# BartvLaatum/GreenLight-Gym2

Measured on AMD Instinct MI355X. Metric: TomatoEnv env-steps/sec, higher is better.
Workload: dtype f32

## Files before the change

greenlight-gym2_amd/csrc/glgym.hip:

```cpp
#include <hip/hip_runtime.h>

#include <cmath>
#include <cstdio>
#include <cstdlib>
#include <cstring>
#include <new>
#include <string>
#include <type_traits>
#include <vector>

#include "glgym.h"
#include "gl_model.hpp"
#include "gl_model_quad.hpp"
#include "gl_reward.hpp"
#include "gl_step_select.hpp"
#include "glgym_bdf.h"
#include "glgym_rng.h"
#include "glgym_plan.h"

using namespace glm;

namespace {

thread_local std::string g_err;

#define HIPCHK(expr)                                                                                   \
    do {                                                                                               \
        hipError_t e_ = (expr);                                                                        \
        if (e_ != hipSuccess) {                                                                        \
            g_err = std::string(#expr) + ": " + hipGetErrorString(e_);                                 \
            return GLGYM_EHIP;                                                                         \
        }                                                                                              \
    } while (0)

constexpr int WAVE = 64;

#include "gl_default_const.inc"
static_assert(sizeof(ModelConst<float>) == sizeof(kDefaultConstF32_image), "regenerate gl_default_const.inc");
static_assert(sizeof(ModelConst<double>) == sizeof(kDefaultConstF64_image), "regenerate gl_default_const.inc");
template <class T> struct DefaultConst;
template <> struct DefaultConst<float> {
    static constexpr ModelConst<float> value = __builtin_bit_cast(ModelConst<float>, kDefaultConstF32_bits);
};
template <> struct DefaultConst<double> {
    static constexpr ModelConst<double> value = __builtin_bit_cast(ModelConst<double>, kDefaultConstF64_bits);
};
__constant__ const ModelConst<float> g_default_f32 = __builtin_bit_cast(ModelConst<float>, kDefaultConstF32_bits);
__constant__ const ModelConst<double> g_default_f64 = __builtin_bit_cast(ModelConst<double>, kDefaultConstF64_bits);
template <class T> __device__ __forceinline__ const ModelConst<T>& device_default();
template <> __device__ __forceinline__ const ModelConst<float>& device_default<float>() { return g_default_f32; }
template <> __device__ __forceinline__ const ModelConst<double>& device_default<double>() { return g_default_f64; }

template <class T> struct RewardConst : RewardConstBase<T> {};

template <class T> struct StepArgsT {
    int B, ld;
    T* x; T* u;
    const float* action; const T* control;
    const T* weather; int weather_rows;
    const int* w_off; int* timestep;
    const T* crop_p;
    int N;
    T* reward; T* info; unsigned char* done; float* metrics; int* step_flags;
    T dt; int n_sub;
    T gasR, tCanMin;
    int nd;
    float du, u_min[NU], u_max[NU];
    int verify;
    int pipe;
    int window;
};

template <class T> __device__ __forceinline__ T wave_sum(T v)
{
#pragma unroll
    for (int o = 32; o > 0; o >>= 1) v += __shfl_xor(v, o, WAVE);
    return v;
}

constexpr int OBS_NCORE = 23;
__device__ __forceinline__ float obs_core_feature(int j, float prim, float aux, float sday, int ts, double doy_inc, double hod_inc)
{
#pragma clang fp contract(off)
    const float kPpm = (float)(8.3144598 / (101325.0 * 44.01e-3));
    const int k = ts > 0 ? ts - 1 : 0;
    const float sat = 610.78f * __builtin_amdgcn_exp2f(1.44269504f * 17.2694f * aux * __builtin_amdgcn_rcpf(aux + 238.3f));
    const float rh = fminf(fmaxf(100.0f * prim * __builtin_amdgcn_rcpf(sat), 0.0f), 100.0f);
    const float ppm = kPpm * (aux + 273.15f) * prim;
    const int c = j - 18;
    const double rev = (c <= 2) ? __builtin_fma((double)ts, doy_inc, (double)sday) * (1.0 / 365.0)
                                : (double)ts * hod_inc * (1.0 / 24.0);
    const float fr = (float)(rev - floor(rev));
    const float clk = (c == 1 || c == 3) ? __builtin_amdgcn_sinf(fr) : __builtin_amdgcn_cosf(fr);
    float v = prim;
    v = (j == 0 || j == 16) ? ppm : v;
    v = (j == 2 || j == 15) ? rh : v;
    v = (j == 18) ? (float)k : v;
    v = (j > 18) ? clk : v;
    return v;
}
__device__ __forceinline__ constexpr int obs_core_module(int j) { return j < 4 ? 0 : j < 7 ? 1 : j < 13 ? 2 : j < 18 ? 3 : 4; }
__device__ __forceinline__ constexpr int obs_core_col(int j) { return j < 4 ? j : j < 7 ? j - 4 : j < 13 ? j - 7 : j < 18 ? j - 13 : j - 18; }

__device__ __forceinline__ void philox4x32_10(unsigned c0, unsigned c1, unsigned c2, unsigned c3, unsigned k0,
                                              unsigned k1, unsigned* out)
{
#pragma unroll
    for (int r = 0; r < 10; ++r) {
        const unsigned long long p0 = 0xD2511F53ull * c0, p1 = 0xCD9E8D57ull * c2;
        const unsigned n0 = (unsigned)(p1 >> 32) ^ c1 ^ k0, n1 = (unsigned)p1;
        const unsigned n2 = (unsigned)(p0 >> 32) ^ c3 ^ k1, n3 = (unsigned)p0;
        c0 = n0; c1 = n1; c2 = n2; c3 = n3;
        k0 += 0x9E3779B9u; k1 += 0xBB67AE85u;
    }
    out[0] = c0; out[1] = c1; out[2] = c2; out[3] = c3;
}

template <class T>
__device__ __forceinline__ void reset_env(int b, int ld, T* x, T* u, int* timestep, const T* weather, int weather_rows, int* w_off,
                                          const int* start_rows, const float* start_days, int n_starts, float* start_day, int* episode,
                                          unsigned long long seed, int nd)
{
#pragma clang fp contract(off)
    if (start_rows && n_starts > 0) {
        const int ep = episode ? episode[b] : 0;
        unsigned rnd[4];
        philox4x32_10((unsigned)b, (unsigned)ep, 0x5eedu, 0u, (unsigned)seed, (unsigned)(seed >> 32), rnd);
        const int j = (int)(rnd[0] % (unsigned)n_starts);
        w_off[b] = start_rows[j];
        if (start_day && start_days) start_day[b] = start_days[j];
        if (episode) episode[b] = ep + 1;
    }
    int r = w_off[b];
    r = r < 0 ? 0 : (r >= weather_rows ? weather_rows - 1 : r);
    const double co2Out = (double)weather[(size_t)r * nd + 3], tSoOut = (double)weather[(size_t)r * nd + 6];
    const double tAir = 16.5;
    double xi[NX];
    xi[0] = xi[1] = co2Out;
    for (int i = 2; i <= 10; ++i) xi[i] = tAir;
    xi[4] = tAir + 4;
    xi[11] = 0.25 * (3.0 * tAir + tSoOut);
    xi[12] = 0.25 * __builtin_fma(2.0, tSoOut, 2.0 * tAir);
    xi[13] = 0.25 * __builtin_fma(3.0, tSoOut, tAir);
    xi[14] = tSoOut;
    xi[15] = xi[16] = 90.0 / 100.0 * (610.78 * exp(17.2694 * tAir / (tAir + 238.3)));
    xi[17] = xi[18] = xi[19] = xi[20] = tAir;
    xi[21] = xi[4];
    xi[22] = 0.0; xi[23] = 9.5283e4; xi[24] = 2.5107e5; xi[25] = 5.5338e4; xi[26] = 3.0978e3; xi[27] = 0.0;
    for (int i = 0; i < NX; ++i) x[(size_t)i * ld + b] = T(xi[i]);
    for (int j = 0; j < NU; ++j) u[(size_t)j * ld + b] = T(0);
    timestep[b] = 0;
}

#ifndef GL_OBS_ROWS
#define GL_OBS_ROWS 16
#endif
constexpr int OBS_ROWS = GL_OBS_ROWS, OBS_MAX_NP = 128;
struct StepObsArgs {
    float* obs; const float* start_day;
    double doy_inc, hod_inc;
    int Np, dim, moff[6];
};
constexpr int STEP_OBS_MAX_DIM_OCC2 = WAVE * ((2 * NX + GL_N_SLOW) | 1) / OBS_ROWS, STEP_OBS_MAX_DIM_OCC1 = 512;
struct StepNoObs {};
struct StepObsResetArgs : StepObsArgs {
    float* term_obs;
    int* w_off_rw; float* start_day_rw; int* episode;
    const int* start_rows; const float* start_days; int n_starts;
    unsigned long long seed;
};
constexpr int GL_SCH_OBS = 8;
constexpr int GL_SCH_RESET = 16;
template <int EPI> struct StepObsSel { using type = StepNoObs; };
template <> struct StepObsSel<GL_SCH_OBS> { using type = StepObsArgs; };
template <> struct StepObsSel<GL_SCH_OBS | GL_SCH_RESET> { using type = StepObsResetArgs; };

#ifndef GL_STEP_WAVES_PER_SIMD
#define GL_STEP_WAVES_PER_SIMD 1
#endif
#ifndef GL_RK4_WIN_F32
#define GL_RK4_WIN_F32 4
#endif
#ifndef GL_RK4_WIN_F64
#define GL_RK4_WIN_F64 4
#endif
template <class T> struct RK4_WINDOW { static constexpr int value = sizeof(T) == 4 ? GL_RK4_WIN_F32 : GL_RK4_WIN_F64; };
constexpr int gl_order(int sch) { return sch == 0 ? 4 : sch == 1 ? 2 : sch == 2 ? 3 : 5; }
template <class T, int SCH> struct SchemeWin { static constexpr int value = SCH == 0 ? RK4_WINDOW<T>::value : SCH == 1 ? 4 : SCH == 2 ? 3 : 2; };

template <class T, bool PER_ENV_CROP, bool DEFAULT_P, bool PIPE = false, int SCHX = 0, int OCC = GL_STEP_WAVES_PER_SIMD>
__global__ __launch_bounds__(WAVE, OCC) void step_kernel(StepArgsT<T> a, ModelConst<T> m_arg, RewardConst<T> rw,
                                                         typename StepObsSel<(SCHX & (GL_SCH_OBS | GL_SCH_RESET))>::type o)
{
    constexpr bool OBS = (SCHX & GL_SCH_OBS) != 0, RST = (SCHX & GL_SCH_RESET) != 0;
    constexpr int SCH = SCHX & (GL_SCH_OBS - 1);
    static_assert(!OBS || (sizeof(T) == 4 && !PIPE), "observation epilogue: fp32, default ODE");
    static_assert(!RST || (OBS && !PER_ENV_CROP), "auto-reset epilogue: behind the observation epilogue, shared crop parameters");
    const ModelConst<T>& m = DEFAULT_P ? device_default<T>() : m_arg;
    constexpr bool WBUF = OCC == 2;
    constexpr int WSTRIDE = (2 * NX + GL_N_SLOW) | 1;
    alignas(16) __shared__ float sh_w[WBUF ? WAVE * WSTRIDE : WAVE * NU];
    float* sh_act = sh_w;
    const int lane = threadIdx.x;
    const int b0 = blockIdx.x * WAVE;
    const int b = b0 + lane;
    const bool live = b < a.B;
    const int bb = live ? b : a.B - 1;

    T u[NU];
    if (a.action) {
        const int n_tile = min(WAVE, a.B - b0) * NU;
        for (int i = lane; i < n_tile; i += WAVE) sh_act[i] = a.action[(size_t)b0 * NU + i];
        __syncthreads();
        const int l = live ? lane : (a.B - 1 - b0);
#pragma unroll
        for (int j = 0; j < NU; ++j) {
            const float inc = sh_act[l * NU + j] * a.du;
            const T v = a.u[(size_t)j * a.ld + bb] + T(inc);
            u[j] = Math<T>::min(Math<T>::max(v, T(a.u_min[j])), T(a.u_max[j]));
        }
    } else {
#pragma unroll
        for (int j = 0; j < NU; ++j) u[j] = a.control[(size_t)j * a.ld + bb];
    }

    T x0[NX];
#pragma unroll
    for (int i = 0; i < NX; ++i) x0[i] = a.x[(size_t)i * a.ld + bb];
    const int ts = a.timestep[bb];
    int row = a.w_off[bb] + ts;
    row = row < 0 ? 0 : (row >= a.weather_rows ? a.weather_rows - 1 : row);
    T d[7];
#pragma unroll
    for (int j = 0; j < 7; ++j) d[j] = a.weather[(size_t)row * a.nd + j];

    CropConst<T> crLocal;
    if (PER_ENV_CROP) {
        T pc[NCROP];
#pragma unroll
        for (int i = 0; i < NCROP; ++i) pc[i] = a.crop_p[(size_t)i * a.ld + bb];
        make_crop_const<T, T>(pc, a.gasR, a.tCanMin, crLocal);
    }
    const CropConst<T>& cr = PER_ENV_CROP ? crLocal : m.crop;
    StepCoef<T> s_reg;
    precompute(u, d, m, cr, s_reg);
    if (PIPE) {
        const T tPipe = a.weather[(size_t)row * a.nd + 10], swOff = a.weather[(size_t)row * a.nd + 12];
        s_reg.pipeTrack = ((tPipe < T(1)) || (swOff > T(0))) ? T(0) : T(1);
        s_reg.tPipeSet = tPipe;
    }
    const StepCoef<T>& s = s_reg;
    if (live) {
#pragma unroll
        for (int j = 0; j < NU; ++j) a.u[(size_t)j * a.ld + b] = u[j];
    }
    T del_reg[WBUF ? 1 : NX];
    T* wb = reinterpret_cast<T*>(sh_w) + (size_t)lane * WSTRIDE;
    T* del = WBUF ? wb + NX + GL_N_SLOW : del_reg;
    if (WBUF) {
        __syncthreads();
#pragma unroll
        for (int i = 0; i < NX; ++i) wb[i] = x0[i];
        wb[5] = x0[3] - x0[5]; wb[7] = x0[2] - x0[7]; wb[20] = x0[2] - x0[20]; wb[6] = x0[5] - x0[6];
    }
    bool bad;
    int extra_steps, first_flags = 0;
    const int retries = rk4_delta_guarded<T, PIPE, gl_order(SCH), SchemeWin<T, SCH>::value, WBUF>(x0, s, m, cr, a.dt, a.n_sub, del, &bad, &extra_steps, a.verify != 0, &first_flags, a.window, wb);
    const T uBoil = a.u[(size_t)0 * a.ld + bb], uCo2 = a.u[(size_t)1 * a.ld + bb], uLamp = a.u[(size_t)4 * a.ld + bb];
    if (WBUF) {
#pragma unroll
        for (int i = 0; i < NX; ++i) x0[i] = a.x[(size_t)i * a.ld + bb];
    }

    T x1[NX];
#pragma unroll
    for (int i = 0; i < NX; ++i) x1[i] = bad ? x0[i] : x0[i] + del[i];
    {
        const double per_step = (double)a.dt / 86400.0;
        double t_start = (double)x0[NX - 1] - (double)ts * per_step;
        if (fabs(t_start) < 5e-4) t_start = 0.0;
        if (!bad) x1[NX - 1] = T(t_start + ((double)ts + 1.0) * per_step);
    }

    const T co2ppm = rw.kPpm * (x1[2] + T(273.15)) * x1[0];
    const T rh = Math<T>::min(Math<T>::max(T(100) * x1[15] / sat_vp_exact(x1[2]), T(0)), T(100));
    const T o3[3] = {co2ppm, x1[2], rh};
    T viol[3], pen = T(0);
#pragma unroll
    for (int i = 0; i < 3; ++i) {
        viol[i] = Math<T>::max(rw.lo[i] - o3[i], T(0)) + Math<T>::max(o3[i] - rw.hi[i], T(0));
        pen += viol[i] * rw.invMaxViol[i];
    }
    const T heat = uBoil * rw.heatK, elec = uLamp * rw.elecK, co2c = uCo2 * rw.co2K;
    const T varc = heat + co2c + elec;
    const T gains = (bad ? T(0) : del[25]) * rw.gainK;
    const T profit = gains - varc;
    const T reward = (profit - rw.minProfit) * rw.invRange - pen;
    const bool term = bad || (ts >= a.N);

    if (live) {
#pragma unroll
        for (int i = 0; i < NX; ++i) a.x[(size_t)i * a.ld + b] = x1[i];
        a.timestep[b] = ts + 1;
        a.reward[b] = reward;
        a.done[b] = term ? 1 : 0;
        if (a.step_flags) a.step_flags[b] = first_flags | (retries << 8) | (bad ? GLGYM_SF_FAILED : 0) | (min(extra_steps, 32767) << 16);
        if (a.info) {
            const T inf[GLGYM_NINFO] = {profit, gains, varc, rw.fixedCosts, co2c, heat, elec, viol[1], viol[0], viol[2], T(0)};
#pragma unroll
            for (int i = 0; i < GLGYM_NINFO; ++i) a.info[(size_t)i * a.ld + b] = inf[i];
        }
    }
    if (a.metrics) {
        const float w = live ? 1.f : 0.f;
        float mv[GLGYM_NMETRIC] = {w * (float)reward, w * (float)profit, (live && term) ? 1.f : 0.f,
                                   (live && bad) ? 1.f : 0.f, w * (float)viol[0], w * (float)viol[1],
                                   w * (float)viol[2], w, w * (float)retries, w * (float)extra_steps,
                                   (live && (first_flags & SC_FLAG_ERR)) ? 1.f : 0.f, (live && (first_flags & SC_FLAG_BRANCH)) ? 1.f : 0.f,
                                   (live && (first_flags & (SC_FLAG_CAP | SC_FLAG_NONFINITE))) ? 1.f : 0.f,
                                   (live && (first_flags & 16)) ? 1.f : 0.f};
        float* mrep = a.metrics + (size_t)(blockIdx.x % GLGYM_METRIC_REPLICAS) * GLGYM_METRIC_STRIDE;
#pragma unroll
        for (int i = 0; i < GLGYM_NMETRIC; ++i) {
            const float sum = wave_sum(mv[i]);
            if (lane == 0) atomicAdd(mrep + i, sum);
        }
    }
    if constexpr (OBS) {
        typedef float v4f __attribute__((ext_vector_type(4)));
        float* span;
        if constexpr (WBUF) {
            span = sh_w;
        } else {
            __shared__ float4 sh_obs4[OBS_ROWS * STEP_OBS_MAX_DIM_OCC1 / 4];
            span = reinterpret_cast<float*>(sh_obs4);
        }
        const int dim = o.dim;
        const int ts1 = ts + 1;
        const int base = a.w_off[bb] + (ts1 > 0 ? ts1 - 1 : 0);
        const int basec = base >= a.weather_rows ? a.weather_rows - 1 : (base < 0 ? 0 : base);
        const T* wrow = a.weather + (size_t)basec * a.nd;
        float wv[5];
#pragma unroll
        for (int j = 0; j < 5; ++j) wv[j] = wrow[j];
        const float sday = o.start_day[bb];
        const float uo[NU] = {uBoil, uCo2, a.u[(size_t)2 * a.ld + bb], a.u[(size_t)3 * a.ld + bb], uLamp, a.u[(size_t)5 * a.ld + bb]};
        float f[OBS_NCORE];
#pragma unroll
        for (int j = 0; j < OBS_NCORE; ++j) {
            const int xi = j == 0 ? 0 : j == 1 ? 2 : j == 2 ? 15 : j == 3 ? 9 : j == 4 ? 21 : j == 5 ? 25 : 26;
            const float prim = j < 7 ? x1[xi] : (j < 13 ? uo[(j >= 7 && j < 13) ? j - 7 : 0] : wv[j < 18 ? j - 13 : 0]);
            const float aux = j < 13 ? x1[2] : wv[1];
            f[j] = obs_core_feature(j, prim, aux, sday, ts1, o.doy_inc, o.hod_inc);
        }
        const int n_live = min(WAVE, a.B - b0);
        const int nf = o.moff[5] >= 0 ? 5 * o.Np : 0;
        __syncthreads();
        for (int s0 = 0; s0 < n_live; s0 += OBS_ROWS) {
            const int nrows = min(OBS_ROWS, n_live - s0);
            const int r_me = lane - s0;
            if (r_me >= 0 && r_me < nrows) {
#pragma unroll
                for (int j = 0; j < OBS_NCORE; ++j) {
                    const int mo = o.moff[obs_core_module(j)];
                    if (mo >= 0) span[r_me * dim + mo + obs_core_col(j)] = f[j];
                }
            }
            int base_r[OBS_ROWS];
#pragma unroll
            for (int r = 0; r < OBS_ROWS; ++r) base_r[r] = __builtin_amdgcn_readlane(base, s0 + r);
            for (int q = lane; q < nf; q += WAVE) {
                const int i = q / 5, c = q - i * 5;
                float v[OBS_ROWS];
#pragma unroll
                for (int r = 0; r < OBS_ROWS; ++r) {
                    int row = base_r[r] + 1 + i;
                    row = row >= a.weather_rows ? a.weather_rows - 1 : (row < 0 ? 0 : row);
                    v[r] = (float)a.weather[(size_t)row * a.nd + c];
                }
#pragma unroll
                for (int r = 0; r < OBS_ROWS; ++r)
                    if (r < nrows) span[r * dim + o.moff[5] + q] = v[r];
            }
            __syncthreads();
            float* out = o.obs + (size_t)(b0 + s0) * dim;
            if (nrows == OBS_ROWS) {
                const int n4 = (OBS_ROWS * dim) >> 2;
                const v4f* src4 = reinterpret_cast<const v4f*>(span);
                v4f* dst4 = reinterpret_cast<v4f*>(out);
                for (int e = lane; e < n4; e += WAVE) __builtin_nontemporal_store(src4[e], &dst4[e]);
            } else {
                for (int r = 0; r < nrows; ++r)
                    for (int jj = lane; jj < dim; jj += WAVE) out[(size_t)r * dim + jj] = span[(size_t)r * dim + jj];
            }
            __syncthreads();
        }
        if constexpr (RST) {
            const bool fin = live && term;
            const unsigned long long fin_mask = __builtin_amdgcn_ballot_w64(fin);
            if (fin_mask != 0) {
                const size_t row0 = (size_t)b0 * dim;
                __syncthreads();
                if (o.term_obs) {
                    for (unsigned long long mk = fin_mask; mk != 0; mk &= mk - 1) {
                        const size_t e0 = row0 + (size_t)__builtin_ctzll(mk) * dim;
                        for (int jj = lane; jj < dim; jj += WAVE) o.term_obs[e0 + jj] = o.obs[e0 + jj];
                    }
                }
                __syncthreads();
                int base_new = 0;
                if (fin) {
                    reset_env<T>(b, a.ld, a.x, a.u, a.timestep, a.weather, a.weather_rows, o.w_off_rw, o.start_rows, o.start_days, o.n_starts,
                                 o.start_day_rw, o.episode, o.seed, a.nd);
                    base_new = o.w_off_rw[b];
                    const int basen = base_new >= a.weather_rows ? a.weather_rows - 1 : (base_new < 0 ? 0 : base_new);
                    const T* wrown = a.weather + (size_t)basen * a.nd;
                    float wn[5];
#pragma unroll
                    for (int j = 0; j < 5; ++j) wn[j] = wrown[j];
                    const float sdayn = o.start_day_rw[b];
                    const float tAirn = a.x[(size_t)2 * a.ld + b];
                    float* orow = o.obs + row0 + (size_t)lane * dim;
#pragma unroll
                    for (int j = 0; j < OBS_NCORE; ++j) {
                        const int xi = j == 0 ? 0 : j == 1 ? 2 : j == 2 ? 15 : j == 3 ? 9 : j == 4 ? 21 : j == 5 ? 25 : 26;
                        const float prim = j < 7 ? a.x[(size_t)xi * a.ld + b] : (j < 13 ? 0.0f : wn[j < 18 ? j - 13 : 0]);
                        const float aux = j < 13 ? tAirn : wn[1];
                        const int mo = o.moff[obs_core_module(j)];
                        if (mo >= 0) orow[mo + obs_core_col(j)] = obs_core_feature(j, prim, aux, sdayn, 0, o.doy_inc, o.hod_inc);
                    }
                }
                for (unsigned long long mk = fin_mask; mk != 0; mk &= mk - 1) {
                    const int r = __builtin_ctzll(mk);
                    const int base_r1 = __builtin_amdgcn_readlane(base_new, r);
                    float* orow = o.obs + row0 + (size_t)r * dim + o.moff[5];
                    for (int q = lane; q < nf; q += WAVE) {
                        const int i = q / 5, c = q - i * 5;
                        int row = base_r1 + 1 + i;
                        row = row >= a.weather_rows ? a.weather_rows - 1 : (row < 0 ? 0 : row);
                        orow[q] = (float)a.weather[(size_t)row * a.nd + c];
                    }
                }
            }
        }
    }
}


template <class T, bool DEFAULT_P, int SCH = 0, bool PIPE = false, bool CROP = false, bool PAIR = false>
__global__ __launch_bounds__(WAVE) void step_kernel_quad(StepArgsT<T> a, ModelConst<T> m_arg, RewardConst<T> rw)
{
    static_assert(!(PAIR && CROP), "the two-rungs ladder is instantiated for shared crop constants only");
    constexpr bool LDSM = sizeof(T) == 8 && !DEFAULT_P;
    __shared__ ModelConst<T> sh_m[1];
    if (LDSM) {
        static_assert(sizeof(ModelConst<T>) % 4 == 0, "word copy");
        const unsigned* src = reinterpret_cast<const unsigned*>(&m_arg);
        unsigned* dst = reinterpret_cast<unsigned*>(&sh_m[0]);
        for (int i = threadIdx.x; i < (int)(sizeof(ModelConst<T>) / 4); i += WAVE) dst[i] = src[i];
        __syncthreads();
    }
    const ModelConst<T>& m = LDSM ? sh_m[0] : DEFAULT_P ? device_default<T>() : m_arg;
    const int gl = blockIdx.x * WAVE + threadIdx.x, role = gl & 3;
    const int b = PAIR ? gl >> 3 : gl >> 2, half = PAIR ? (gl >> 2) & 1 : 0;
    const bool live = b < a.B;
    const int bb = live ? b : a.B - 1;
    T u[NU];
    if (a.action) {
#pragma unroll
        for (int j = 0; j < NU; ++j) {
            const float inc = a.action[(size_t)bb * NU + j] * a.du;
            const T v = a.u[(size_t)j * a.ld + bb] + T(inc);
            u[j] = Math<T>::min(Math<T>::max(v, T(a.u_min[j])), T(a.u_max[j]));
        }
    } else {
#pragma unroll
        for (int j = 0; j < NU; ++j) u[j] = a.control[(size_t)j * a.ld + bb];
    }
    const int ts = a.timestep[bb];
    int row = a.w_off[bb] + ts;
    row = row < 0 ? 0 : (row >= a.weather_rows ? a.weather_rows - 1 : row);
    T d[7];
#pragma unroll
    for (int j = 0; j < 7; ++j) d[j] = a.weather[(size_t)row * a.nd + j];
    constexpr bool LDSQ = sizeof(T) == 8;
    struct SRec { StepCoef<T> s; T pad[(sizeof(StepCoef<T>) / sizeof(T)) % 2 == 0 ? 1 : 2]; };
    struct KRec { LaneK<T> k; T pad[(sizeof(LaneK<T>) / sizeof(T)) % 2 == 0 ? 1 : 2]; };
    struct CRec { CropConst<T> c; T pad[(sizeof(CropConst<T>) / sizeof(T)) % 2 == 0 ? 1 : 2]; };
    __shared__ SRec sh_s[LDSQ ? WAVE / 4 : 1];
    __shared__ KRec sh_k[LDSQ ? WAVE : 1];
    __shared__ CRec sh_c[(LDSQ && CROP) ? WAVE / 4 : 1];
    StepCoef<T> s_reg;
    LaneK<T> k_reg;
    CropConst<T> cr_reg;
    if (CROP && (!LDSQ || role == 0)) {
        T pc[NCROP];
#pragma unroll
        for (int i = 0; i < NCROP; ++i) pc[i] = a.crop_p[(size_t)i * a.ld + bb];
        make_crop_const<T, T>(pc, a.gasR, a.tCanMin, cr_reg);
    }
    if (!LDSQ || role == 0) {
        precompute(u, d, m, CROP ? cr_reg : m.crop, s_reg);
        if (PIPE && a.pipe) {
            const T tPipe = a.weather[(size_t)row * a.nd + 10], swOff = a.weather[(size_t)row * a.nd + 12];
            s_reg.pipeTrack = ((tPipe < T(1)) || (swOff > T(0))) ? T(0) : T(1);
            s_reg.tPipeSet = tPipe;
            s_reg.pipeOde = T(1);
        }
    }
    if (LDSQ) {
        if (role == 0) { sh_s[threadIdx.x >> 2].s = s_reg; if (CROP) sh_c[threadIdx.x >> 2].c = cr_reg; }
        __syncthreads();
    }
    const CropConst<T>& cr = !CROP ? m.crop : LDSQ ? sh_c[threadIdx.x >> 2].c : cr_reg;
    const StepCoef<T>& s = LDSQ ? sh_s[threadIdx.x >> 2].s : s_reg;
    LaneK<T>& K = LDSQ ? sh_k[threadIdx.x].k : k_reg;
    auto X = [&](int i) { return a.x[(size_t)i * a.ld + bb]; };
    QVec<T> x0, z0, del;
#pragma unroll
    for (int i = 0; i < 6; ++i) x0.sh[i] = X(role == 0 ? gq_sh_ix(i) : role == 1 ? gq_sh_ix(i) : role == 2 ? gq_sh_ix(i) : gq_sh_ix(i));
    x0.p = gq_mk<T>(X(role == 0 ? 4 : role == 1 ? 8 : role == 2 ? 7 : 5), X(role == 0 ? 9 : role == 1 ? 17 : role == 2 ? 20 : 6));
#pragma unroll
    for (int j = 0; j < 4; ++j) {
        const int ix = role == 0 ? gq_other_ix(0, j) : role == 1 ? gq_other_ix(1, j) : role == 2 ? gq_other_ix(2, j) : gq_other_ix(3, j < 2 ? j : 1);
        x0.o[j] = X(ix);
    }
    z0 = x0;
    z0.p = gq_mk<T>(role == 2 ? x0.sh[2] - x0.p.x : role == 3 ? x0.sh[3] - x0.p.x : x0.p.x,
                    role == 2 ? x0.sh[2] - x0.p.y : role == 3 ? x0.p.x - x0.p.y : x0.p.y);
    if (live && role == 0 && half == 0) {
#pragma unroll
        for (int j = 0; j < NU; ++j) a.u[(size_t)j * a.ld + b] = u[j];
    }
    bool bad;
    int extra_steps = 0, first_flags = 0, retries = 0, mine = 1;
    constexpr bool HVU = sizeof(T) == 8 || DEFAULT_P;
    if (PAIR) {
        int bad_i;
        rk4_delta_guarded_quad_pair<T, gl_order(SCH), SchemeWin<T, SCH>::value, LDSQ, PIPE, false, true, HVU>(role, half, z0, s, K, m, cr, a.dt, a.n_sub, del, &bad_i, &mine,
                                                                                                         a.window, &retries, &extra_steps, &first_flags);
        asm volatile("" : "+v"(bad_i), "+v"(mine));
        bad = bad_i != 0;
    } else {
        retries = rk4_delta_guarded_quad<T, gl_order(SCH), SchemeWin<T, SCH>::value, LDSQ, PIPE, LDSQ && CROP, HVU>(role, z0, s, K, m, cr, a.dt, a.n_sub, del, &bad,
                                                                                                    &extra_steps, a.verify != 0, &first_flags, a.window);
    }
    P2<T> dP;
    gq_phys_pair<T>(role, del, dP);
    asm volatile("" ::: "memory");
    int gl2 = blockIdx.x * WAVE + threadIdx.x;
    asm volatile("" : "+v"(gl2));
    const int role2 = gl2 & 3, b2 = PAIR ? gl2 >> 3 : gl2 >> 2;
    const bool live2 = b2 < a.B && mine != 0;
    const int bb2 = (b2 < a.B) ? b2 : a.B - 1;
    const int ts2 = a.timestep[bb2];
    auto X2 = [&](int i) { return a.x[(size_t)i * a.ld + bb2]; };
#pragma unroll
    for (int i = 0; i < 6; ++i) x0.sh[i] = X2(gq_sh_ix(i));
    x0.p = gq_mk<T>(X2(role2 == 0 ? 4 : role2 == 1 ? 8 : role2 == 2 ? 7 : 5), X2(role2 == 0 ? 9 : role2 == 1 ? 17 : role2 == 2 ? 20 : 6));
#pragma unroll
    for (int j = 0; j < 4; ++j) {
        const int ix = role2 == 0 ? gq_other_ix(0, j) : role2 == 1 ? gq_other_ix(1, j) : role2 == 2 ? gq_other_ix(2, j) : gq_other_ix(3, j < 2 ? j : 1);
        x0.o[j] = X2(ix);
    }
#pragma unroll
    for (int j = 0; j < NU; ++j) u[j] = a.u[(size_t)j * a.ld + bb2];
    QVec<T> x1;
    x1.p = gq_mk<T>(bad ? x0.p.x : x0.p.x + dP.x, bad ? x0.p.y : x0.p.y + dP.y);
#pragma unroll
    for (int i = 0; i < 6; ++i) x1.sh[i] = bad ? x0.sh[i] : x0.sh[i] + del.sh[i];
#pragma unroll
    for (int j = 0; j < 4; ++j) x1.o[j] = bad ? x0.o[j] : x0.o[j] + del.o[j];
    if (role2 == 3) {
        const double per_step = (double)a.dt / 86400.0;
        double t_start = (double)x0.o[1] - (double)ts2 * per_step;
        if (fabs(t_start) < 5e-4) t_start = 0.0;
        if (!bad) x1.o[1] = T(t_start + ((double)ts2 + 1.0) * per_step);
    }
    const T dFruit = gq_bcast<2>(del.o[3]);
    const T co2ppm = rw.kPpm * (x1.sh[2] + T(273.15)) * x1.sh[0];
    const T rh = Math<T>::min(Math<T>::max(T(100) * x1.sh[4] / sat_vp_exact(x1.sh[2]), T(0)), T(100));
    const T o3[3] = {co2ppm, x1.sh[2], rh};
    T viol[3], pen = T(0);
#pragma unroll
    for (int i = 0; i < 3; ++i) {
        viol[i] = Math<T>::max(rw.lo[i] - o3[i], T(0)) + Math<T>::max(o3[i] - rw.hi[i], T(0));
        pen += viol[i] * rw.invMaxViol[i];
    }
    const T heat = u[0] * rw.heatK, elec = u[4] * rw.elecK, co2c = u[1] * rw.co2K;
    const T varc = heat + co2c + elec;
    const T gains = (bad ? T(0) : dFruit) * rw.gainK;
    const T profit = gains - varc;
    const T reward = (profit - rw.minProfit) * rw.invRange - pen;
    const bool term = bad || (ts2 >= a.N);
    if (live2) {
        auto W = [&](int i, T v) { a.x[(size_t)i * a.ld + b2] = v; };
        W(role2 == 0 ? 4 : role2 == 1 ? 8 : role2 == 2 ? 7 : 5, x1.p.x);
        W(role2 == 0 ? 9 : role2 == 1 ? 17 : role2 == 2 ? 20 : 6, x1.p.y);
#pragma unroll
        for (int j = 0; j < 4; ++j)
            if (role2 != 3 || j < 2) W(role2 == 0 ? gq_other_ix(0, j) : role2 == 1 ? gq_other_ix(1, j) : role2 == 2 ? gq_other_ix(2, j) : gq_other_ix(3, j < 2 ? j : 1), x1.o[j]);
        if (role2 == 0) {
#pragma unroll
            for (int i = 0; i < 6; ++i) W(gq_sh_ix(i), x1.sh[i]);
            a.timestep[b2] = ts2 + 1;
            a.reward[b2] = reward;
            a.done[b2] = term ? 1 : 0;
            if (a.step_flags) a.step_flags[b2] = first_flags | (retries << 8) | (bad ? GLGYM_SF_FAILED : 0) | (min(extra_steps, 32767) << 16);
            if (a.info) {
                const T inf[GLGYM_NINFO] = {profit, gains, varc, rw.fixedCosts, co2c, heat, elec, viol[1], viol[0], viol[2], T(0)};
#pragma unroll
                for (int i = 0; i < GLGYM_NINFO; ++i) a.info[(size_t)i * a.ld + b2] = inf[i];
            }
        }
    }
    if (a.metrics) {
        const bool cnt = live2 && role2 == 0;
        const float w = cnt ? 1.f : 0.f;
        float mv[GLGYM_NMETRIC] = {w * (float)reward, w * (float)profit, (cnt && term) ? 1.f : 0.f,
                                   (cnt && bad) ? 1.f : 0.f, w * (float)viol[0], w * (float)viol[1],
                                   w * (float)viol[2], w, w * (float)retries, w * (float)extra_steps,
                                   (cnt && (first_flags & SC_FLAG_ERR)) ? 1.f : 0.f, (cnt && (first_flags & SC_FLAG_BRANCH)) ? 1.f : 0.f,
                                   (cnt && (first_flags & (SC_FLAG_CAP | SC_FLAG_NONFINITE))) ? 1.f : 0.f,
                                   (cnt && (first_flags & 16)) ? 1.f : 0.f};
        float* mrep = a.metrics + (size_t)(blockIdx.x % GLGYM_METRIC_REPLICAS) * GLGYM_METRIC_STRIDE;
#pragma unroll
        for (int i = 0; i < GLGYM_NMETRIC; ++i) {
            const float sum = wave_sum(mv[i]);
            if (threadIdx.x == 0) atomicAdd(mrep + i, sum);
        }
    }
}

template <class T, int SCH, bool PIPE, bool CROP, bool PAIR = false>
__global__ __launch_bounds__(WAVE) void evalf_kernel_quad(const double* x, const double* u, const double* d, const double* crop, int B, T dt,
                                                          int n_sub, T gasR, T tCanMin, ModelConst<T> m_arg, double* x_next, int nd,
                                                          int* n_failed, int verify, int pipe, int window)
{
    constexpr bool LDSM = sizeof(T) == 8;
    __shared__ ModelConst<T> sh_m[1];
    if (LDSM) {
        const unsigned* src = reinterpret_cast<const unsigned*>(&m_arg);
        unsigned* dst = reinterpret_cast<unsigned*>(&sh_m[0]);
        for (int i = threadIdx.x; i < (int)(sizeof(ModelConst<T>) / 4); i += WAVE) dst[i] = src[i];
        __syncthreads();
    }
    const ModelConst<T>& m = LDSM ? sh_m[0] : m_arg;
    const int gl = blockIdx.x * WAVE + threadIdx.x, role = gl & 3, b = PAIR ? gl >> 3 : gl >> 2, half = PAIR ? (gl >> 2) & 1 : 0;
    const bool live = b < B;
    const int bb = live ? b : B - 1;
    T uu[NU], dd[7];
#pragma unroll
    for (int i = 0; i < NU; ++i) uu[i] = T(u[(size_t)bb * NU + i]);
#pragma unroll
    for (int i = 0; i < 7; ++i) dd[i] = T(d[(size_t)bb * nd + i]);
    constexpr bool LDSQ = sizeof(T) == 8;
    struct SRec { StepCoef<T> s; T pad[(sizeof(StepCoef<T>) / sizeof(T)) % 2 == 0 ? 1 : 2]; };
    struct KRec { LaneK<T> k; T pad[(sizeof(LaneK<T>) / sizeof(T)) % 2 == 0 ? 1 : 2]; };
    struct CRec { CropConst<T> c; T pad[(sizeof(CropConst<T>) / sizeof(T)) % 2 == 0 ? 1 : 2]; };
    __shared__ SRec sh_s[LDSQ ? WAVE / 4 : 1];
    __shared__ KRec sh_k[LDSQ ? WAVE : 1];
    __shared__ CRec sh_c[(LDSQ && CROP) ? WAVE / 4 : 1];
    StepCoef<T> s_reg;
    LaneK<T> k_reg;
    CropConst<T> cr_reg;
    if (CROP && (!LDSQ || role == 0)) {
        T pc[NCROP];
#pragma unroll
        for (int i = 0; i < NCROP; ++i) pc[i] = T(crop[(size_t)bb * NCROP + i]);
        make_crop_const<T, T>(pc, gasR, tCanMin, cr_reg);
    }
    if (!LDSQ || role == 0) {
        precompute(uu, dd, m, CROP ? cr_reg : m.crop, s_reg);
        if (PIPE && pipe) {
            const T tPipe = T(d[(size_t)bb * nd + 10]), swOff = T(d[(size_t)bb * nd + 12]);
            s_reg.pipeTrack = ((tPipe < T(1)) || (swOff > T(0))) ? T(0) : T(1);
            s_reg.tPipeSet = tPipe;
            s_reg.pipeOde = T(1);
        }
    }
    if (LDSQ) {
        if (role == 0) { sh_s[threadIdx.x >> 2].s = s_reg; if (CROP) sh_c[threadIdx.x >> 2].c = cr_reg; }
        __syncthreads();
    }
    const CropConst<T>& cr = !CROP ? m.crop : LDSQ ? sh_c[threadIdx.x >> 2].c : cr_reg;
    const StepCoef<T>& s = LDSQ ? sh_s[threadIdx.x >> 2].s : s_reg;
    LaneK<T>& K = LDSQ ? sh_k[threadIdx.x].k : k_reg;
    auto X = [&](int i) { return T(x[(size_t)bb * NX + i]); };
    QVec<T> x0, z0, del;
#pragma unroll
    for (int i = 0; i < 6; ++i) x0.sh[i] = X(gq_sh_ix(i));
    x0.p = gq_mk<T>(X(role == 0 ? 4 : role == 1 ? 8 : role == 2 ? 7 : 5), X(role == 0 ? 9 : role == 1 ? 17 : role == 2 ? 20 : 6));
#pragma unroll
    for (int j = 0; j < 4; ++j)
        x0.o[j] = X(role == 0 ? gq_other_ix(0, j) : role == 1 ? gq_other_ix(1, j) : role == 2 ? gq_other_ix(2, j) : gq_other_ix(3, j < 2 ? j : 1));
    z0 = x0;
    z0.p = gq_mk<T>(role == 2 ? x0.sh[2] - x0.p.x : role == 3 ? x0.sh[3] - x0.p.x : x0.p.x,
                    role == 2 ? x0.sh[2] - x0.p.y : role == 3 ? x0.p.x - x0.p.y : x0.p.y);
    bool bad;
    constexpr bool HVU = sizeof(T) == 8;
    int mine = 1;
    if (PAIR) {
        int bad_i;
        rk4_delta_guarded_quad_pair<T, gl_order(SCH), SchemeWin<T, SCH>::value, LDSQ, PIPE, LDSQ && CROP, false, HVU>(role, half, z0, s, K, m, cr, dt, n_sub, del, &bad_i, &mine, window);
        asm volatile("" : "+v"(bad_i), "+v"(mine));
        bad = bad_i != 0;
    } else {
        int extra_steps, first_flags = 0;
        rk4_delta_guarded_quad<T, gl_order(SCH), SchemeWin<T, SCH>::value, LDSQ, PIPE, LDSQ && CROP, HVU>(role, z0, s, K, m, cr, dt, n_sub, del, &bad, &extra_steps, verify != 0,
                                                                                      &first_flags, window);
    }
    P2<T> dP;
    gq_phys_pair<T>(role, del, dP);
    asm volatile("" ::: "memory");
    int gl2 = blockIdx.x * WAVE + threadIdx.x;
    asm volatile("" : "+v"(gl2));
    const int role2 = gl2 & 3, b2 = PAIR ? gl2 >> 3 : gl2 >> 2;
    if (b2 < B && mine != 0) {
        const double nan = __builtin_nan("");
        auto X2 = [&](int i) { return x[(size_t)b2 * NX + i]; };
        auto W = [&](int i, T dv) { x_next[(size_t)b2 * NX + i] = bad ? nan : X2(i) + (double)dv; };
        W(role2 == 0 ? 4 : role2 == 1 ? 8 : role2 == 2 ? 7 : 5, dP.x);
        W(role2 == 0 ? 9 : role2 == 1 ? 17 : role2 == 2 ? 20 : 6, dP.y);
#pragma unroll
        for (int j = 0; j < 4; ++j)
            if (role2 != 3 || j < 2)
                W(role2 == 0 ? gq_other_ix(0, j) : role2 == 1 ? gq_other_ix(1, j) : role2 == 2 ? gq_other_ix(2, j) : gq_other_ix(3, j < 2 ? j : 1), del.o[j]);
        if (role2 == 0) {
#pragma unroll
            for (int i = 0; i < 6; ++i) W(gq_sh_ix(i), del.sh[i]);
            if (bad) atomicAdd(n_failed, 1);
        }
    }
}

template <class T, bool PER_ENV_CROP, bool PIPE>
__global__ __launch_bounds__(WAVE) void rhs_kernel(const double* x, const double* u, const double* d, const double* crop, int B, T gasR,
                                                   T tCanMin, ModelConst<T> m, double* dx, int nd)
{
    const int b = blockIdx.x * WAVE + threadIdx.x;
    if (b >= B) return;
    T x0[NX], uu[NU], dd[7];
    for (int i = 0; i < NX; ++i) x0[i] = T(x[(size_t)b * NX + i]);
    for (int i = 0; i < NU; ++i) uu[i] = T(u[(size_t)b * NU + i]);
// ... 1557 lines not shown
```

Baseline: 104.3 million.

## Write observations directly to global memory, bypassing the LDS staging buffer

Each lane now stores its core observation features straight to its own global obs row. The forecast weather block is copied by groups of 8 rows with precomputed per-lane offsets and no clamping, software-pipelined with double-buffered registers. Only groups whose forecast windows cross the weather bounds fall back to a per-row clamped copy. This removes the shared-memory staging, the __syncthreads barriers and the per-element clamp arithmetic, at the cost of scattered scalar stores instead of coalesced float4 stores and higher register use.

```diff
diff --git a/greenlight-gym2_amd/csrc/glgym.hip b/greenlight-gym2_amd/csrc/glgym.hip
--- a/greenlight-gym2_amd/csrc/glgym.hip
+++ b/greenlight-gym2_amd/csrc/glgym.hip
@@ -175,6 +175,87 @@
 template <> struct StepObsSel<GL_SCH_OBS> { using type = StepObsArgs; };
 template <> struct StepObsSel<GL_SCH_OBS | GL_SCH_RESET> { using type = StepObsResetArgs; };
 
+template <int R, int KC>
+__device__ __forceinline__ void obs_fc_load(float (&v)[R][KC], const float* weather, int nd, const int (&first)[R], const unsigned (&foff)[KC])
+{
+#pragma unroll
+    for (int r = 0; r < R; ++r) {
+        const char* w0 = reinterpret_cast<const char*>(weather + (ptrdiff_t)first[r] * nd);
+#pragma unroll
+        for (int k = 0; k < KC; ++k) v[r][k] = *reinterpret_cast<const float*>(w0 + foff[k]);
+    }
+}
+template <int R, int KC>
+__device__ __forceinline__ void obs_fc_store(const float (&v)[R][KC], float* const* out, int lane, int nf)
+{
+#pragma unroll
+    for (int r = 0; r < R; ++r) {
+#pragma unroll
+        for (int k = 0; k < KC - 1; ++k) __builtin_nontemporal_store(v[r][k], out[r] + lane + WAVE * k);
+    }
+    if (lane + WAVE * (KC - 1) < nf) {
+#pragma unroll
+        for (int r = 0; r < R; ++r) __builtin_nontemporal_store(v[r][KC - 1], out[r] + lane + WAVE * (KC - 1));
+    }
+}
+template <int R, int KC>
+__device__ __forceinline__ void obs_fc_groups(unsigned fast, const float* weather, int nd, int first, float* out0, int dim, int lane, int nf)
+{
+    unsigned foff[KC];
+#pragma unroll
+    for (int k = 0; k < KC; ++k) {
+        const int q = min(lane + WAVE * k, nf - 1);
+        const int i = q / 5;
+        foff[k] = (unsigned)(i * nd + (q - i * 5)) * 4u;
+    }
+    auto load = [&](int g, float (&v)[R][KC]) {
+        int fr[R];
+#pragma unroll
+        for (int r = 0; r < R; ++r) fr[r] = __builtin_amdgcn_readlane(first, g * R + r);
+        obs_fc_load(v, weather, nd, fr, foff);
+    };
+    auto store = [&](int g, const float (&v)[R][KC]) {
+        float* out[R];
+#pragma unroll
+        for (int r = 0; r < R; ++r) out[r] = out0 + (size_t)(g * R + r) * dim;
+        obs_fc_store(v, out, lane, nf);
+    };
+    auto next = [&]() { const int g = __builtin_ctz(fast); fast &= fast - 1; return g; };
+    if (fast == 0) return;
+    float va[R][KC], vb[R][KC];
+    int ga = next(), gb;
+    load(ga, va);
+    for (;;) {
+        if (fast == 0) { store(ga, va); break; }
+        gb = next();
+        load(gb, vb);
+        store(ga, va);
+        if (fast == 0) { store(gb, vb); break; }
+        ga = next();
+        load(ga, va);
+        store(gb, vb);
+    }
+}
+template <int R, int KC>
+__device__ __forceinline__ bool obs_fc_dispatch(int kc, unsigned fast, const float* weather, int nd, int first, float* out0, int dim, int lane, int nf)
+{
+    if (kc == KC) {
+        obs_fc_groups<R, KC>(fast, weather, nd, first, out0, dim, lane, nf);
+        return true;
+    }
+    if constexpr (KC > 1) return obs_fc_dispatch<R, KC - 1>(kc, fast, weather, nd, first, out0, dim, lane, nf);
+    return false;
+}
+__device__ __forceinline__ void obs_fc_row_clamped(const float* weather, int weather_rows, int nd, int first, float* out, int lane, int nf)
+{
+    for (int q = lane; q < nf; q += WAVE) {
+        const int i = q / 5, c = q - i * 5;
+        int row = first + i;
+        row = row >= weather_rows ? weather_rows - 1 : (row < 0 ? 0 : row);
+        __builtin_nontemporal_store(weather[(size_t)row * nd + c], out + q);
+    }
+}
+
 #ifndef GL_STEP_WAVES_PER_SIMD
 #define GL_STEP_WAVES_PER_SIMD 1
 #endif
@@ -327,13 +408,10 @@
         }
     }
     if constexpr (OBS) {
-        typedef float v4f __attribute__((ext_vector_type(4)));
-        float* span;
-        if constexpr (WBUF) {
-            span = sh_w;
-        } else {
+        constexpr int FC_ROWS = 8, FC_KMAX = ((WBUF ? STEP_OBS_MAX_DIM_OCC2 : STEP_OBS_MAX_DIM_OCC1) + WAVE - 1) / WAVE;
+        if constexpr (!WBUF) {
             __shared__ float4 sh_obs4[OBS_ROWS * STEP_OBS_MAX_DIM_OCC1 / 4];
-            span = reinterpret_cast<float*>(sh_obs4);
+            asm volatile("" ::"s"((unsigned)(size_t)&sh_obs4[0]));
         }
         const int dim = o.dim;
         const int ts1 = ts + 1;
@@ -355,45 +433,27 @@
         }
         const int n_live = min(WAVE, a.B - b0);
         const int nf = o.moff[5] >= 0 ? 5 * o.Np : 0;
-        __syncthreads();
-        for (int s0 = 0; s0 < n_live; s0 += OBS_ROWS) {
-            const int nrows = min(OBS_ROWS, n_live - s0);
-            const int r_me = lane - s0;
-            if (r_me >= 0 && r_me < nrows) {
-#pragma unroll
-                for (int j = 0; j < OBS_NCORE; ++j) {
-                    const int mo = o.moff[obs_core_module(j)];
-                    if (mo >= 0) span[r_me * dim + mo + obs_core_col(j)] = f[j];
-                }
+        if (live) {
+            float* orow = o.obs + (size_t)b * dim;
+#pragma unroll
+            for (int j = 0; j < OBS_NCORE; ++j) {
+                const int mo = o.moff[obs_core_module(j)];
+                if (mo >= 0) __builtin_nontemporal_store(f[j], orow + mo + obs_core_col(j));
             }
-            int base_r[OBS_ROWS];
-#pragma unroll
-            for (int r = 0; r < OBS_ROWS; ++r) base_r[r] = __builtin_amdgcn_readlane(base, s0 + r);
-            for (int q = lane; q < nf; q += WAVE) {
-                const int i = q / 5, c = q - i * 5;
-                float v[OBS_ROWS];
-#pragma unroll
-                for (int r = 0; r < OBS_ROWS; ++r) {
-                    int row = base_r[r] + 1 + i;
-                    row = row >= a.weather_rows ? a.weather_rows - 1 : (row < 0 ? 0 : row);
-                    v[r] = (float)a.weather[(size_t)row * a.nd + c];
-                }
-#pragma unroll
-                for (int r = 0; r < OBS_ROWS; ++r)
-                    if (r < nrows) span[r * dim + o.moff[5] + q] = v[r];
-            }
-            __syncthreads();
-            float* out = o.obs + (size_t)(b0 + s0) * dim;
-            if (nrows == OBS_ROWS) {
-                const int n4 = (OBS_ROWS * dim) >> 2;
-                const v4f* src4 = reinterpret_cast<const v4f*>(span);
-                v4f* dst4 = reinterpret_cast<v4f*>(out);
-                for (int e = lane; e < n4; e += WAVE) __builtin_nontemporal_store(src4[e], &dst4[e]);
-            } else {
-                for (int r = 0; r < nrows; ++r)
-                    for (int jj = lane; jj < dim; jj += WAVE) out[(size_t)r * dim + jj] = span[(size_t)r * dim + jj];
-            }
-            __syncthreads();
+        }
+        if (nf > 0) {
+            const int first = base + 1;
+            const unsigned long long leaves = __builtin_amdgcn_ballot_w64(live && (first < 0 || first + o.Np > a.weather_rows));
+            const int kc = (nf + WAVE - 1) / WAVE;
+            unsigned fast = 0;
+#pragma unroll
+            for (int g = 0; g < WAVE / FC_ROWS; ++g)
+                if ((g + 1) * FC_ROWS <= n_live && ((leaves >> (g * FC_ROWS)) & ((1ull << FC_ROWS) - 1)) == 0) fast |= 1u << g;
+            float* const out0 = o.obs + (size_t)b0 * dim + o.moff[5];
+            if (!obs_fc_dispatch<FC_ROWS, FC_KMAX>(kc, fast, a.weather, a.nd, first, out0, dim, lane, nf)) fast = 0;
+            for (int r = 0; r < n_live; ++r)
+                if (!((fast >> (r / FC_ROWS)) & 1))
+                    obs_fc_row_clamped(a.weather, a.weather_rows, a.nd, __builtin_amdgcn_readlane(first, r), out0 + (size_t)r * dim, lane, nf);
         }
         if constexpr (RST) {
             const bool fin = live && term;
@@ -432,14 +492,8 @@
                 }
                 for (unsigned long long mk = fin_mask; mk != 0; mk &= mk - 1) {
                     const int r = __builtin_ctzll(mk);
-                    const int base_r1 = __builtin_amdgcn_readlane(base_new, r);
-                    float* orow = o.obs + row0 + (size_t)r * dim + o.moff[5];
-                    for (int q = lane; q < nf; q += WAVE) {
-                        const int i = q / 5, c = q - i * 5;
-                        int row = base_r1 + 1 + i;
-                        row = row >= a.weather_rows ? a.weather_rows - 1 : (row < 0 ? 0 : row);
-                        orow[q] = (float)a.weather[(size_t)row * a.nd + c];
-                    }
+                    obs_fc_row_clamped(a.weather, a.weather_rows, a.nd, __builtin_amdgcn_readlane(base_new, r) + 1,
+                                       o.obs + row0 + (size_t)r * dim + o.moff[5], lane, nf);
                 }
             }
         }
```

After: 104.8 million, median of 6. Within noise of the previous version (+0.5%).
